# paplorinc/jtokkit

Hardware: AMD Instinct MI355X
Metric: input MB/s encoded (cl100k_base), HBM-resident input and output, bit-exact vs CPU oracle (higher is better)
Workload: dtype int32; 1 GPU; cl100k_base, 1M mixed UTF-8 docs (emoji + CJK, ~4 KB each); docs=1000000, bytes=4099377688, docs_per_gpu=1000000, bytes_per_gpu=4099377688, encode=encode() incl. the special-token check

## Files before the change

### jtokkit_amd/csrc/jtk_kernels.hip

```cpp
#include "jtk_kernels.h"

#include <type_traits>

#include "jtk_device_prims.h"
#include "jtk_merge_core.h"
#include "jtk_merge_order_rules.h"
#include "jtk_block_classify.h"
#include "jtk_split_masks.h"
#include "jtk_split_rules.h"

namespace {

constexpr int WAVE = 64;

__device__ __forceinline__ uint64_t lanemask_lt() {
    const unsigned lane = threadIdx.x & 63u;
    return (1ull << lane) - 1ull;
}

__device__ __forceinline__ void wave_lds_fence() {
    __builtin_amdgcn_fence(__ATOMIC_RELEASE, "wavefront");
    __builtin_amdgcn_wave_barrier();
    __builtin_amdgcn_fence(__ATOMIC_ACQUIRE, "wavefront");
}
// ... 1213 lines not shown
        uint32_t r = JTK_RANK_NONE;
        if (lane == 0 && nn >= 0) r = jtk_pair_lookup(pt, minr, ids[nn]);
        if (lane == 1 && pv >= 0) r = jtk_pair_lookup(pt, ids[pv], minr);
        wave_lds_fence();
        if (lane == 0) { ids[mini] = minr; rk[mini] = r; ids[nxt] = JTK_ID_DEAD; }
        if (lane == 1 && pv >= 0) rk[pv] = r;
        wave_lds_fence();
    }
}

template <int CAP>
__device__ __forceinline__ void merge_long(const JtkWork& w, const JtkDeviceTables& t, uint32_t* s_id, uint32_t* s_rk,
                                           uint32_t wave_id, uint32_t n_waves) {
    const int lane = threadIdx.x & 63;
    const JtkLongPiece* list = (CAP == JTK_MID_CAP) ? w.mid_list : w.long_list;
    const uint32_t cnt = (CAP == JTK_MID_CAP) ? *w.mid_count : *w.long_count;
    for (uint32_t i = wave_id; i < cnt; i += n_waves) {
        const JtkLongPiece lp = list[i];
        if (lp.len <= 0) continue;
        const int len = (int)lp.len;
        for (int j = lane; j < len; j += WAVE) {
            const uint32_t b0 = w.text[lp.start + j];
            s_id[j] = t.byte_rank[b0];
            s_rk[j] = (j + 1 < len) ? t.bp_rank[(b0 << 8) | w.text[lp.start + j + 1]] : JTK_RANK_NONE;
        }
        wave_lds_fence();
        merge_piece_wave(s_id, s_rk, len, t.pairs);
        uint32_t total = 0;
        for (int base = 0; base < len; base += WAVE) {
            const int j = base + lane;
            const bool alive = j < len && s_id[j] != JTK_ID_DEAD;
            const uint64_t bal = __ballot(alive);
            const uint32_t idx = total + (uint32_t)__popcll(bal & lanemask_lt());
            if (alive && idx) w.htok[lp.start + idx] = s_id[j];
            total += (uint32_t)__popcll(bal);
        }
        if (lane == 0) {
            w.htok[lp.start] = s_id[0] | (total << JTK_HT_CNT_SHIFT);
            atomicAdd(&w.tile_tot[lp.start / T], total);
        }
        wave_lds_fence();
    }
}

__device__ __forceinline__ uint64_t wave_min_u64(uint64_t v) {
#pragma unroll
    for (int d = 1; d < 64; d <<= 1) {
        const uint32_t lo = (uint32_t)__shfl_xor((int)(uint32_t)v, d), hi = (uint32_t)__shfl_xor((int)(uint32_t)(v >> 32), d);
        const uint64_t o = ((uint64_t)hi << 32) | lo;
        v = o < v ? o : v;
    }
    return v;
}

struct GiantLds {
    uint64_t* cmin;
    uint64_t* wmin;
    int* nb;
    uint32_t* r;
};

__device__ void merge_giant(const JtkWork& w, const JtkDeviceTables& t, const GiantLds& L, uint32_t gi) {
    constexpr int CH = JTK_GIANT_CHUNK;
    const int tid = threadIdx.x, lane = tid & 63, wv = tid >> 6, NT = blockDim.x, NWV = NT >> 6;
    const JtkLongPiece lp = w.giant_list[gi];
    if (lp.len <= 0) return;
    const int len = (int)lp.len;
    uint32_t* gid = w.htok + lp.start;
    uint32_t* grk = w.docpre + lp.start;
    const int nch = (len + CH - 1) / CH;
    constexpr uint64_t KNONE = ~0ull;

    for (int j = tid; j < len; j += NT) {
        const uint32_t b0 = w.text[lp.start + j];
        gid[j] = t.byte_rank[b0];
        grk[j] = (j + 1 < len) ? t.bp_rank[(b0 << 8) | w.text[lp.start + j + 1]] : JTK_RANK_NONE;
    }
    __syncthreads();
    auto chunk_min = [&](int c) {
        uint64_t k = KNONE;
        for (int q = 0; q < CH / 64; q++) {
            const int j = c * CH + q * 64 + lane;
            if (j < len) { const uint32_t r = grk[j]; if (r != JTK_RANK_NONE) { const uint64_t kk = ((uint64_t)r << 20) | (uint32_t)j; k = kk < k ? kk : k; } }
        }
        k = wave_min_u64(k);
        if (lane == 0) L.cmin[c] = k;
    };
    for (int c = wv; c < nch; c += NWV) chunk_min(c);
    __syncthreads();

    for (;;) {
        uint64_t k = KNONE;
        for (int c = tid; c < nch; c += NT) { const uint64_t kk = L.cmin[c]; k = kk < k ? kk : k; }
        k = wave_min_u64(k);
        if (lane == 0) L.wmin[wv] = k;
        __syncthreads();
        k = L.wmin[0];
        for (int q = 1; q < NWV; q++) k = L.wmin[q] < k ? L.wmin[q] : k;
        if (k == KNONE) break;
        const uint32_t minr = (uint32_t)(k >> 20);
        const int mini = (int)(k & 0xFFFFFu);
        if (wv == 0) {
            int nxt = -1, nn = -1;
            for (int base = mini + 1; base < len && nn < 0; base += WAVE) {
                const int j = base + lane;
                uint64_t bal = __ballot(j < len && gid[j] != JTK_ID_DEAD);
                if (nxt < 0 && bal) { nxt = base + jtk_ctz64(bal); bal &= bal - 1; }
                if (nxt >= 0 && bal) nn = base + jtk_ctz64(bal);
            }
            if (lane == 0) { L.nb[0] = nxt; L.nb[1] = nn; L.r[0] = nn >= 0 ? jtk_pair_lookup(t.pairs, minr, gid[nn]) : JTK_RANK_NONE; }
        } else if (wv == 1) {
            int pv = -1;
            for (int base = mini - 1; base >= 0 && pv < 0; base -= WAVE) {
                const int j = base - lane;
                const uint64_t bal = __ballot(j >= 0 && gid[j] != JTK_ID_DEAD);
                if (bal) pv = base - jtk_ctz64(bal);
            }
            if (lane == 0) { L.nb[2] = pv; L.r[1] = pv >= 0 ? jtk_pair_lookup(t.pairs, gid[pv], minr) : JTK_RANK_NONE; }
        }
        __syncthreads();
        const int nxt = L.nb[0], pv = L.nb[2];
        if (tid == 0) {
            gid[mini] = minr; grk[mini] = L.r[0];
            gid[nxt] = JTK_ID_DEAD; grk[nxt] = JTK_RANK_NONE;
            if (pv >= 0) grk[pv] = L.r[1];
        }
        __syncthreads();
        const int c0 = mini / CH, c1 = nxt / CH, c2 = pv >= 0 ? pv / CH : c0;
        if (wv == 0) chunk_min(c0);
        if (wv == 1 && c1 != c0) chunk_min(c1);
        if (wv == 2 && c2 != c0 && c2 != c1) chunk_min(c2);
        __syncthreads();
    }
    if (wv == 0) {
        uint32_t total = 0;
        uint32_t first = 0;
        for (int base = 0; base < len; base += WAVE) {
            const int j = base + lane;
            const uint32_t v = j < len ? gid[j] : JTK_ID_DEAD;
            const bool alive = v != JTK_ID_DEAD;
            const uint64_t bal = __ballot(alive);
            const uint32_t idx = total + (uint32_t)__popcll(bal & lanemask_lt());
            if (base == 0) first = (uint32_t)__shfl((int)v, 0);
            if (alive && idx) gid[idx] = v;
            total += (uint32_t)__popcll(bal);
        }
        if (lane == 0) {
            gid[0] = first | ((uint32_t)JTK_HT_ESCAPE << JTK_HT_CNT_SHIFT);
            grk[1] = total;
            atomicAdd(&w.tile_tot[lp.start / T], total);
        }
    }
    __syncthreads();
}

__global__ void __launch_bounds__(ML_THREADS) k_bpe_merge(JtkWork w, JtkDeviceTables t) {
    __shared__ alignas(16) uint32_t s_id[ML_WORDS];
    __shared__ alignas(16) uint32_t s_rk[ML_WORDS];
    __shared__ uint64_t s_bpbits[1024];
    __shared__ uint32_t s_bpranks[JTK_BP_MAX];
    __shared__ uint16_t s_bpcum[1024];
    __shared__ uint32_t s_brank[256];
    __shared__ uint32_t s_next[JTK_NBINS];
    __shared__ uint32_t s_count[JTK_NBINS + 3];
    __shared__ uint32_t s_ntiny;
    const int tid = threadIdx.x;
    const int shard = blockIdx.x % JTK_Q_SHARDS;
    const uint32_t kq = blockIdx.x / JTK_Q_SHARDS;
    if (tid < JTK_NBINS) {
        s_next[tid] = 0;
        s_count[tid] = w.q_count[JTK_QC(tid, shard)];
    }
    if (tid == 16) s_ntiny = w.q_count[JTK_QC(JTK_BIN_TINY, shard)];
    if (tid == JTK_NBINS) s_count[JTK_NBINS] = *w.mid_count;
    if (tid == JTK_NBINS + 1) s_count[JTK_NBINS + 1] = *w.long_count;
    if (tid == JTK_NBINS + 2) s_count[JTK_NBINS + 2] = *w.n_giant;
    __syncthreads();
    const uint32_t n0 = s_count[0], n1 = s_count[1], n2 = s_count[2], n3 = s_count[3], n4 = s_count[4];
    const uint32_t nt5 = s_ntiny;
    const bool rest = (s_count[5] | s_count[6] | s_count[JTK_NBINS] | s_count[JTK_NBINS + 1] | s_count[JTK_NBINS + 2]) != 0u;
    const bool side_by_side = n0 <= (uint32_t)ML_THREADS && n1 <= (uint32_t)ML_THREADS && n2 <= (uint32_t)ML_THREADS &&
                              nt5 <= (uint32_t)ML_THREADS && n3 <= (uint32_t)(ML_THREADS / 2) && n4 <= (uint32_t)(ML_THREADS / 4) &&
                              gridDim.x / JTK_Q_SHARDS >= 4u;
    const uint32_t K = side_by_side ? 1u : gridDim.x / JTK_Q_SHARDS, k = side_by_side ? 0u : kq;
    bool w0, w1, w2, w3, w4, w5;
    if (side_by_side) {
        w0 = kq == 0u && n0; w1 = kq == 1u && n1; w2 = kq == 2u && n2;
        w5 = kq == 3u && nt5; w3 = kq == 3u && n3; w4 = kq == 3u && n4;
    } else {
        w0 = kq * (uint32_t)ML_THREADS < n0; w1 = kq * (uint32_t)ML_THREADS < n1; w2 = kq * (uint32_t)ML_THREADS < n2;
        w3 = kq * (uint32_t)(ML_THREADS / 2) < n3; w4 = kq * (uint32_t)(ML_THREADS / 4) < n4;
        w5 = kq * (uint32_t)ML_THREADS < nt5;
    }
    if (!(w0 || w1 || w2 || w3 || w4 || w5 || rest)) return;
    for (int i = tid; i < 1024; i += ML_THREADS) { s_bpbits[i] = t.bp.bits[i]; s_bpcum[i] = t.bp.cum[i]; }
    for (int i = tid; i < JTK_BP_MAX; i += ML_THREADS) s_bpranks[i] = t.bp.ranks[i];
    if (tid < 256) s_brank[tid] = t.byte_rank[tid];
    __syncthreads();
    const LeanLds LL{s_id, s_rk, JtkBpLds{s_bpbits, s_bpcum, s_bpranks}, s_brank};
    if (w5) tiny_bin<ML_THREADS>(w, LL, nt5, k, K);
    if (w0) lean_bin<16, ML_THREADS, 0>(w, t, LL, n0, k, K);
    if (w1) lean_bin<16, ML_THREADS, 1>(w, t, LL, n1, k, K);
    if (w2) lean_bin<16, ML_THREADS, 2>(w, t, LL, n2, k, K);
    if (w3) { __syncthreads(); lean_bin<32, ML_THREADS / 2, 3>(w, t, LL, n3, k, K); }
    if (w4) { __syncthreads(); lean_bin<64, ML_THREADS / 4, 4>(w, t, LL, n4, k, K); }
    if (!rest) return;
    const MergeLds L{s_id, s_rk, s_bpbits, s_bpranks, s_bpcum, s_brank, s_next, s_count};
    if (s_count[5]) { __syncthreads(); merge_bin<128, ML_WORDS / 128, 5>(w, t, L); }
    if (s_count[6]) { __syncthreads(); merge_bin<256, ML_WORDS / 256, 6>(w, t, L); }
    const uint32_t wv = (uint32_t)tid >> 6;
    if (s_count[JTK_NBINS]) {
        __syncthreads();
        merge_long<JTK_MID_CAP>(w, t, s_id + wv * JTK_MID_CAP, s_rk + wv * JTK_MID_CAP, blockIdx.x * (uint32_t)(ML_THREADS / 64) + wv,
                                gridDim.x * (uint32_t)(ML_THREADS / 64));
    }
    if (s_count[JTK_NBINS + 1]) {
        __syncthreads();
        if (wv == 0) merge_long<JTK_LONG_CAP>(w, t, s_id, s_rk, blockIdx.x, gridDim.x);
    }
    if (s_count[JTK_NBINS + 2]) {
        __syncthreads();
        const GiantLds G{reinterpret_cast<uint64_t*>(s_id), reinterpret_cast<uint64_t*>(s_rk), reinterpret_cast<int*>(s_rk + 64),
                         s_rk + 72};
        for (uint32_t gi = blockIdx.x; gi < s_count[JTK_NBINS + 2]; gi += gridDim.x) merge_giant(w, t, G, gi);
    }
}

constexpr int SCAN_CHUNK = 4096;

__global__ void __launch_bounds__(1024) k_tile_scan(JtkWork w) {
    __shared__ uint64_t s_part[16];
    __shared__ uint32_t s_wsum[16];
    const int tid = threadIdx.x, lane = tid & 63, wv = tid >> 6;
    const int64_t chunk = blockIdx.x;
    uint64_t b = 0;
    {
        const int64_t nb = chunk * SCAN_CHUNK;
        const uint4* t4 = reinterpret_cast<const uint4*>(w.tile_tot);
        for (int64_t i = tid; i < nb / 4; i += 1024) { const uint4 v = t4[i]; b += (uint64_t)v.x + v.y + v.z + v.w; }
    }
    for (int d = 32; d >= 1; d >>= 1) {
        const uint32_t lo = (uint32_t)__shfl_xor((int)(uint32_t)b, d), hi = (uint32_t)__shfl_xor((int)(uint32_t)(b >> 32), d);
        b += ((uint64_t)hi << 32) | lo;
    }
    if (lane == 0) s_part[wv] = b;
    const int64_t i0 = chunk * SCAN_CHUNK + (int64_t)tid * 4;
    uint32_t v[4];
    uint32_t sum = 0;
    for (int j = 0; j < 4; j++) { v[j] = (i0 + j < w.n_tiles) ? w.tile_tot[i0 + j] : 0u; sum += v[j]; }
    const uint32_t inc = jtk_wave_incl_scan(sum);
    if (lane == 63) s_wsum[wv] = inc;
    __syncthreads();
    const uint64_t job_before = (uint64_t)*w.job_tokens;
    uint64_t before = job_before;
    for (int k = 0; k < 16; k++) before += s_part[k];
    for (int k = 0; k < wv; k++) before += s_wsum[k];
    uint64_t run = before + inc - sum;
    for (int j = 0; j < 4; j++) { if (i0 + j < w.n_tiles) w.tile_off[i0 + j] = (int64_t)run; run += v[j]; }
    if (chunk == gridDim.x - 1 && tid == 1023) {
        w.tile_off[w.n_tiles] = (int64_t)run;
        w.set_info[0] = (int64_t)job_before;
        w.set_info[1] = (int64_t)run;
        w.result->n_tokens = (int64_t)run;
        *w.job_tokens_next = (int64_t)run;
    }
}

__device__ __forceinline__ uint32_t hard_count(const JtkWork& w, int64_t pos) {
    const uint32_t c = (w.htok[pos] >> JTK_HT_CNT_SHIFT) & JTK_HT_CNT_MASK;
    if (c != JTK_HT_ESCAPE) return c;
    return w.docpre[pos + 1];
}

template <typename P> __device__ __forceinline__ P* uniform_ptr(P* p) {
    const uint64_t v = reinterpret_cast<uint64_t>(p);
    return reinterpret_cast<P*>((uint64_t)(uint32_t)__builtin_amdgcn_readfirstlane((int)(uint32_t)v) |
                                (uint64_t)(uint32_t)__builtin_amdgcn_readfirstlane((int)(uint32_t)(v >> 32)) << 32);
}

struct __attribute__((packed, aligned(4))) U4Unaligned { uint32_t x, y, z, w; };
__device__ __forceinline__ void pack_copy(uint32_t* dst, const uint32_t* src, uint32_t c) {
    for (uint32_t i = 0; i < c; i += 8) {
        const U4Unaligned a = *reinterpret_cast<const U4Unaligned*>(src + i), b = *reinterpret_cast<const U4Unaligned*>(src + i + 4);
        dst[i] = a.x & JTK_HT_ID_MASK;
        if (i + 1 < c) dst[i + 1] = a.y & JTK_HT_ID_MASK;
        if (i + 2 < c) dst[i + 2] = a.z & JTK_HT_ID_MASK;
        if (i + 3 < c) dst[i + 3] = a.w & JTK_HT_ID_MASK;
        if (i + 4 < c) dst[i + 4] = b.x & JTK_HT_ID_MASK;
        if (i + 5 < c) dst[i + 5] = b.y & JTK_HT_ID_MASK;
        if (i + 6 < c) dst[i + 6] = b.z & JTK_HT_ID_MASK;
        if (i + 7 < c) dst[i + 7] = b.w & JTK_HT_ID_MASK;
    }
}

template <int I> __device__ __forceinline__ uint32_t res_tok(const uint4& r) {
    constexpr int bit = 17 * I, wd = bit / 32, sh = bit % 32;
    const uint32_t w0 = wd == 0 ? r.x : wd == 1 ? r.y : wd == 2 ? r.z : r.w;
    const uint32_t w1 = wd == 0 ? r.y : wd == 1 ? r.z : r.w;
    return (sh + 17 <= 32 ? (w0 >> sh) : __builtin_amdgcn_alignbit(w1, w0, sh)) & JTK_HT_ID_MASK;
}

constexpr int PACK_STAGE = JTK_PACK_STAGE;
constexpr int PQT = JTK_PACK_TINY;

__global__ void __launch_bounds__(64) k_pack_tokens(JtkWork w) {
    __shared__ uint4 s_qe[JTK_PACK_SLOTS + JTK_PACK_OUT_SLOTS];
    __shared__ uint2 s_qt[PQT];
    __shared__ uint64_t s_dm[TW];
    __shared__ uint32_t s_ext[8];
    uint32_t* const s_out = reinterpret_cast<uint32_t*>(s_qe + JTK_PACK_SLOTS);
    const int lane = threadIdx.x;
    const int64_t tile = blockIdx.x;
    const int64_t B = tile * T;
    const int np = (int)w.tile_np[tile];
    const uint32_t total = w.tile_tot[tile];
    const uint32_t meta = lane < 16 ? w.q_meta[tile * 16 + lane] : 0u;
    const bool stage = total <= (uint32_t)PACK_STAGE;
    const bool store = w.count_only == 0;
    const uint32_t* plist = w.plist + B;
    int64_t tile_base;
    if (w.inline_scan) {
        uint32_t part = 0;
        for (int64_t i = lane; i < tile; i += 64) part += w.tile_tot[i];
#pragma unroll
        for (int d = 32; d >= 1; d >>= 1) part += (uint32_t)__shfl_xor((int)part, d);
        const int64_t job_before = *w.job_tokens;
        tile_base = job_before + (int64_t)part;
        if (lane == 0) {
            w.tile_off[tile] = tile_base;
            if (tile == w.n_tiles - 1) {
                const int64_t end = tile_base + (int64_t)total;
                w.tile_off[w.n_tiles] = end;
                w.set_info[0] = job_before;
                w.set_info[1] = end;
                w.result->n_tokens = end;
                *w.job_tokens_next = end;
            }
        }
    } else tile_base = w.tile_off[tile];
    uint32_t* const dst = reinterpret_cast<uint32_t*>(w.tokens + tile_base);
    uint32_t e[8];
#pragma unroll
    for (int j = 0; j < 8; j++) e[j] = plist[j * 64 + lane];
    uint64_t dmw = 0ull;
    if (lane < TW) {
        const int64_t dwd = (B >> 6) + lane;
        if (dwd < w.n_words) dmw = w.docmask[dwd];
    }
    const int64_t shard = tile % JTK_Q_SHARDS;
    uint4 rh = make_uint4(0, 0, 0, 0), rl = make_uint4(0, 0, 0, 0);
    bool hv, lv = false;
    {
        const int bl = lane < 32 ? 0 : lane < 48 ? 1 : 2, il = lane < 32 ? lane : lane < 48 ? lane - 32 : lane - 48;
        const uint32_t qbv = (uint32_t)__shfl((int)meta, bl), nqv = (uint32_t)__shfl((int)meta, 8 + bl);
        const uint4* const p0 = uniform_ptr(w.qd[0] + shard * w.q_cap[0]), * const p1 = uniform_ptr(w.qd[1] + shard * w.q_cap[1]),
                   * const p2 = uniform_ptr(w.qd[2] + shard * w.q_cap[2]);
        const uint4* src = (bl == 0 ? p0 : bl == 1 ? p1 : p2) + qbv;
        hv = (uint32_t)il < nqv;
        if (hv) rh = src[il];
    }
    const uint32_t nq_hi = (uint32_t)__shfl((int)meta, 11) | (uint32_t)__shfl((int)meta, 12) | (uint32_t)__shfl((int)meta, 13) | (uint32_t)__shfl((int)meta, 14);
    if (nq_hi) {
        const int bq = 3 + ((lane >> 3) & 3), il = lane & 7;
        const uint32_t qb = (uint32_t)__shfl((int)meta, bq), nq = (uint32_t)__shfl((int)meta, 8 + bq);
        lv = lane < 32 && (uint32_t)il < nq;
        const uint4* const p3 = uniform_ptr(w.qd[3] + shard * w.q_cap[3]), * const p4 = uniform_ptr(w.qd[4] + shard * w.q_cap[4]),
                   * const p5 = uniform_ptr(w.qd[5] + shard * w.q_cap[5]), * const p6 = uniform_ptr(w.qd[6] + shard * w.q_cap[6]);
        if (lv) rl = ((bq == 3 ? p3 : bq == 4 ? p4 : bq == 5 ? p5 : p6) + qb)[il];
    }
    const uint32_t qb5 = (uint32_t)__shfl((int)meta, JTK_BIN_TINY), nq5 = (uint32_t)__shfl((int)meta, 8 + JTK_BIN_TINY);
    const uint2* const res5 = reinterpret_cast<const uint2*>(w.qt + shard * w.qt_cap + qb5);
    uint2 rt[PQT / 64];
    if (nq5) {
#pragma unroll
        for (int r = 0; r < PQT / 64; r++) {
            const uint32_t i = (uint32_t)(r * 64 + lane);
            rt[r] = make_uint2(0, 0);
            if (i < nq5) rt[r] = res5[i];
        }
    }
    constexpr int XR = JTK_PACK_OUT_SLOTS / 64;
    const uint32_t over = (lane >= 8 && lane < 8 + JTK_NBINS_STAGE) ? jtk_stage_over(lane - 8, meta) : 0u;
    const bool has_ext = __ballot(over != 0u) != 0ull;
    uint4 rx[XR];
    uint32_t xend = 0;
    const uint32_t x0 = (uint32_t)JTK_PACK_SLOTS + jtk_stage_first_free(total);
    if (has_ext) {
        const uint32_t inc = jtk_wave_incl_scan(over);
        uint32_t xoff, xn;
        jtk_stage_place(total, inc - over, over, &xoff, &xn);
        if (lane >= 8 && lane < 16) s_ext[lane - 8] = lane < 8 + JTK_NBINS_STAGE ? jtk_stage_word(lane - 8, xoff, xn) : 0u;
        xend = (uint32_t)__builtin_amdgcn_readlane((int)(xoff + xn), 8 + JTK_NBINS_STAGE - 1);
#pragma unroll
        for (int r = 0; r < XR; r++) {
            rx[r] = make_uint4(0, 0, 0, 0);
            if (x0 + r * 64 >= xend) break;
            const uint32_t slot = x0 + r * 64 + lane;
            const uint4* src = nullptr;
#pragma unroll
            for (int b = 0; b < JTK_NBINS_STAGE; b++) {
                const uint32_t n = (uint32_t)__builtin_amdgcn_readlane((int)xn, 8 + b);
                if (n == 0u) continue;
                const uint32_t o = (uint32_t)__builtin_amdgcn_readlane((int)xoff, 8 + b), qb = (uint32_t)__builtin_amdgcn_readlane((int)meta, b);
                const uint4* base = w.qd[b] + shard * w.q_cap[b] + qb + JTK_PACK_CAP(b);
                src = slot - o < n ? base + (slot - o) : src;
            }
            if (slot < xend) rx[r] = *src;
        }
    }
    if (lane < TW) s_dm[lane] = dmw;
    if (hv) s_qe[lane] = rh;
    if (nq_hi) { if (lv) s_qe[JTK_PACK_OFF(3) + lane] = rl; }
    if (nq5) {
#pragma unroll
        for (int r = 0; r < PQT / 64; r++) {
            const uint32_t i = (uint32_t)(r * 64 + lane);
            if (i < nq5) s_qt[i] = rt[r];
        }
    }
    if (has_ext) {
#pragma unroll
        for (int r = 0; r < XR; r++) {
            const uint32_t slot = x0 + r * 64 + lane;
            if (slot < xend) s_qe[slot] = rx[r];
        }
    }
#pragma unroll
    for (int j = 0; j < 8; j++) e[j] = (j * 64 + lane < np) ? e[j] : 0u;
    wave_lds_fence();
    uint32_t run = 0;
    auto tiny_word = [](uint2 r) { return make_uint4(r.x, r.y & 0x3FFFFFFFu, 0u, (r.y >> 30) << 24); };
#define STORE(x) do { if (store) { x; } } while (0)
    auto step = [&](uint32_t* out, uint32_t ej, int k) {
        const bool valid = k < np;
        const bool hard = (ej & JTK_PL_HARD) != 0;
        const uint32_t bin = (ej >> JTK_PL_BIN_SHIFT) & 7u, qi = (ej >> JTK_PL_QI_SHIFT) & 1023u;
        const bool queued = hard && !(ej & JTK_PL_NOQUEUE);
        const bool tinyp = bin == JTK_BIN_TINY;
        const bool staged = queued && (ej & JTK_PL_STAGED) != 0u;
        uint32_t sidx = staged && !tinyp ? qi : 0u;
        bool inlds = staged;
        if (has_ext) {
            const uint32_t xw = s_ext[bin];
            const bool x = queued && !staged && qi < (xw >> 16);
            sidx = x ? (xw & 0xFFFFu) + qi : sidx;
            inlds = staged || x;
        }
        uint4 qe = s_qe[sidx];
        if (__ballot(queued && tinyp)) { if (staged && tinyp) qe = tiny_word(s_qt[qi]); }
        uint32_t c = valid ? (hard ? (qe.w >> 24) + 1u : 1u) : 0u;
        const uint32_t off = hard ? (ej & 2047u) : ((ej >> JTK_PL_OFF_SHIFT) & 2047u);
        const bool isdoc = valid && ((s_dm[off >> 6] >> (off & 63)) & 1ull);
        uint32_t pre;
        if (!__ballot(valid && hard && (!inlds || c > 7u))) {
            const uint32_t x = c ? c - 1u : 0u;
            const uint64_t bv = __ballot(valid);
            const uint64_t b0 = __ballot((x & 1u) != 0u), b1 = __ballot((x & 2u) != 0u), b2 = __ballot((x & 4u) != 0u);
            auto below = [](uint64_t m, uint32_t acc) { return __builtin_amdgcn_mbcnt_hi((uint32_t)(m >> 32), __builtin_amdgcn_mbcnt_lo((uint32_t)m, acc)); };
            pre = below(b0, below(bv, run));
            run += (uint32_t)__popcll(bv) + (uint32_t)__popcll(b0);
            if (b1 | b2) {
                pre += 2u * below(b1, 0u) + 4u * below(b2, 0u);
                run += 2u * (uint32_t)__popcll(b1) + 4u * (uint32_t)__popcll(b2);
            }
            if (valid) STORE(out[pre] = (hard ? qe.x : ej) & JTK_HT_ID_MASK);
            if (b0 | b1 | b2) {
                if (c > 1u) STORE(out[pre + 1] = res_tok<1>(qe));
                if (c > 2u) STORE(out[pre + 2] = res_tok<2>(qe));
                if (b1 | b2) {
                    if (c > 3u) STORE(out[pre + 3] = res_tok<3>(qe));
                    if (b2) {
                        if (c > 4u) STORE(out[pre + 4] = res_tok<4>(qe));
                        if (c > 5u) STORE(out[pre + 5] = res_tok<5>(qe));
                        if (c > 6u) STORE(out[pre + 6] = res_tok<6>(qe));
                    }
                }
            }
        } else {
            const uint32_t qb = (uint32_t)__shfl((int)meta, (int)(bin < JTK_NBINS ? bin : 0u));
            if (valid && queued && !inlds) {
                qe = tinyp ? tiny_word(res5[qi]) : (w.qd[bin] + shard * w.q_cap[bin] + qb)[qi];
                c = (qe.w >> 24) + 1u;
            } else if (valid && hard && !queued) c = hard_count(w, B + off);
            const uint32_t inc = jtk_wave_incl_scan(c);
            pre = run + inc - c;
            run += (uint32_t)__shfl((int)inc, 63);
            if (valid) {
                if (!hard) STORE(out[pre] = ej & JTK_HT_ID_MASK);
                else if (queued && c <= 7u) {
                    STORE(out[pre] = qe.x & JTK_HT_ID_MASK);
                    if (c > 1u) STORE(out[pre + 1] = res_tok<1>(qe));
                    if (c > 2u) STORE(out[pre + 2] = res_tok<2>(qe));
                    if (c > 3u) STORE(out[pre + 3] = res_tok<3>(qe));
                    if (c > 4u) STORE(out[pre + 4] = res_tok<4>(qe));
                    if (c > 5u) STORE(out[pre + 5] = res_tok<5>(qe));
                    if (c > 6u) STORE(out[pre + 6] = res_tok<6>(qe));
                } else if (store) pack_copy(out + pre, w.htok + B + off, c);
            }
        }
        if (__ballot(isdoc)) { if (isdoc) w.docpre[B + off] = pre; }
    };
#undef STORE
    for (int k0 = 0; k0 < np; k0 += 512) {
        if (k0) {
#pragma unroll
            for (int j = 0; j < 8; j++) { const int k = k0 + j * 64 + lane; e[j] = (k < np) ? plist[k] : 0u; }
        }
#pragma unroll
        for (int j = 0; j < 8; j++) {
            if (k0 + j * 64 >= np) break;
            if (stage) step(s_out, e[j], k0 + j * 64 + lane);
            else step(dst, e[j], k0 + j * 64 + lane);
        }
    }
    if (stage && store) {
        wave_lds_fence();
        for (uint32_t i = lane; i < total; i += WAVE) dst[i] = s_out[i];
    }
}

__global__ void __launch_bounds__(256) k_doc_offsets(JtkWork w) {
    const int64_t d = (int64_t)blockIdx.x * blockDim.x + threadIdx.x;
    if (d > w.n_docs) return;
    const int64_t q = w.doc_off[d] - w.text_base;
    w.tok_off[d] = (q >= w.n_bytes || q < w.lead) ? w.tile_off[w.n_tiles] : w.tile_off[q / T] + w.docpre[q];
    if (d < w.n_docs) {
        const int32_t st = w.status[d];
        if (st < 0) atomicMin(&w.result->worst_status, st);
    }
}

__device__ uint32_t long_lookup(const JtkWork& w, const JtkDeviceTables& t, int64_t pos, int64_t len) {
    if (len > (int64_t)t.longtok.max_len || len <= 16) return JTK_RANK_NONE;
    uint64_t h = JTK_FNV_BASIS;
    for (int64_t j = 0; j < len; j++) h = jtk_fnv1a_step(h, w.text[pos + j]);
    const uint32_t n = t.longtok.n;
    for (uint32_t i = (uint32_t)(h % n), probes = 0; probes < n; i = (i + 1) % n, probes++) {
        const JtkLongTokSlot sl = t.longtok.slots[i];
        if (sl.len == 0) return JTK_RANK_NONE;
        if (sl.h_lo == (uint32_t)h && sl.h_hi == (uint32_t)(h >> 32) && sl.len == (uint32_t)len) {
            bool eq = true;
            for (int64_t j = 0; j < len && eq; j++) eq = t.longtok.blob[sl.blob_off + j] == w.text[pos + j];
            if (eq) return sl.id;
        }
    }
    return JTK_RANK_NONE;
}

__global__ void __launch_bounds__(256) k_long_shortcut(JtkWork w, JtkDeviceTables t) {
    const uint32_t gtid = blockIdx.x * blockDim.x + threadIdx.x, gn = gridDim.x * blockDim.x;
    for (int bin = JTK_NBINS_BYTES; bin < JTK_NBINS; bin++) {
        for (int shard = 0; shard < JTK_Q_SHARDS; shard++) {
            const uint32_t count = w.q_count[JTK_QC(bin, shard)];
            uint64_t* qm = w.qm[bin] + (int64_t)shard * w.q_cap[bin];
            uint4* qd = w.qd[bin] + (int64_t)shard * w.q_cap[bin];
            for (uint32_t i = gtid; i < count; i += gn) {
                const uint64_t meta = qm[i];
                const int64_t pos = (int64_t)(meta & JTK_QE_POS_MASK);
                const uint32_t id = long_lookup(w, t, pos, (int64_t)((meta >> JTK_QE_LEN_SHIFT) & 255u) + 1);
                if (id != JTK_RANK_NONE) {
                    qd[i] = make_uint4(id, 0u, 0u, 0u);
                    qm[i] = meta | JTK_QE_DONE;
                    atomicAdd(&w.tile_tot[pos / T], 1u);
                }
            }
        }
    }
    for (int which = 0; which < 3; which++) {
        JtkLongPiece* list = which == 0 ? w.mid_list : which == 1 ? w.long_list : w.giant_list;
        const uint32_t count = which == 0 ? *w.mid_count : which == 1 ? *w.long_count : *w.n_giant;
        for (uint32_t i = gtid; i < count; i += gn) {
            const JtkLongPiece lp = list[i];
            const uint32_t id = long_lookup(w, t, lp.start, lp.len);
            if (id != JTK_RANK_NONE) {
                w.htok[lp.start] = id | (1u << JTK_HT_CNT_SHIFT);
                list[i].len = 0;
                atomicAdd(&w.tile_tot[lp.start / T], 1u);
            }
        }
    }
}

}

__global__ void __launch_bounds__(256) k_plan_chunks(const int64_t* doc_off, int64_t n_docs, int64_t chunk_bytes, int n_chunks,
                                                     int64_t* out_doc, int64_t* out_off) {
    const int c = (int)(blockIdx.x * blockDim.x + threadIdx.x);
    if (c > n_chunks) return;
    const int64_t lo = c == n_chunks ? n_docs : jtk_first_ge(doc_off, 0, n_docs, (int64_t)c * chunk_bytes);
    out_doc[c] = lo;
    out_off[c] = doc_off[lo];
}

void jtk_launch_plan_chunks(const int64_t* doc_off, int64_t n_docs, int64_t chunk_bytes, int n_chunks, int64_t* out_doc, int64_t* out_off,
                            hipStream_t s) {
    hipLaunchKernelGGL(k_plan_chunks, dim3((unsigned)((n_chunks + 1 + 255) / 256)), dim3(256), 0, s, doc_off, n_docs, chunk_bytes, n_chunks,
                       out_doc, out_off);
}

__global__ void __launch_bounds__(256) k_stitch(const int64_t* totals, int rank, int64_t* base_out, const int64_t* tok_off, int64_t n_docs,
                                                int64_t* global_off) {
    int64_t base = 0;
    for (int r = 0; r < rank; r++) base += totals[r];
    const int64_t d = (int64_t)blockIdx.x * blockDim.x + threadIdx.x;
    if (d == 0) *base_out = base;
    if (global_off && d <= n_docs) global_off[d] = tok_off[d] + base;
}
void jtk_launch_stitch(const int64_t* totals, int rank, int64_t* base_out, const int64_t* tok_off, int64_t n_docs, int64_t* global_off,
                       hipStream_t s) {
    const int64_t n = global_off ? n_docs + 1 : 1;
    hipLaunchKernelGGL(k_stitch, dim3((unsigned)((n + 255) / 256)), dim3(256), 0, s, totals, rank, base_out, tok_off, n_docs, global_off);
}

__global__ void __launch_bounds__(256) k_mark_pieces(JtkWork w, const int64_t* begin, const int64_t* end, int64_t n_pieces) {
    const int64_t i = (int64_t)blockIdx.x * blockDim.x + threadIdx.x;
    if (i >= n_pieces) return;
    const int64_t p = begin[i] - w.text_base, e = end[i] - w.text_base;
    if (p < w.lead || e <= p || e > w.n_bytes || (i + 1 < n_pieces && begin[i + 1] - w.text_base < e)) {
        atomicMin(&w.result->worst_status, -1 );
        return;
    }
    atomicOr((unsigned long long*)&w.piecemask[p >> 6], 1ull << (p & 63));
    const bool next_adjacent = (i + 1 < n_pieces) && (begin[i + 1] - w.text_base == e);
    if (!next_adjacent && e < w.n_bytes) {
        atomicOr((unsigned long long*)&w.piecemask[e >> 6], 1ull << (e & 63));
        atomicOr((unsigned long long*)&w.gapmask[e >> 6], 1ull << (e & 63));
    }
}
__global__ void __launch_bounds__(256) k_mark_doc_gaps(JtkWork w) {
    const int64_t d = (int64_t)blockIdx.x * blockDim.x + threadIdx.x;
    if (d > w.n_docs) return;
    const int64_t q = w.doc_off[d] - w.text_base;
    if (q < w.lead || q > w.n_bytes) return;
    const uint64_t bit = 1ull << (q & 63);
    const uint64_t old = atomicOr((unsigned long long*)&w.piecemask[q >> 6], bit);
    if (!(old & bit) && q < w.n_bytes) atomicOr((unsigned long long*)&w.gapmask[q >> 6], bit);
}
void jtk_launch_mark_pieces(const JtkWork& w, const int64_t* begin, const int64_t* end, int64_t n_pieces, hipStream_t s) {
    if (n_pieces > 0)
        hipLaunchKernelGGL(k_mark_pieces, dim3((unsigned)((n_pieces + 255) / 256)), dim3(256), 0, s, w, begin, end, n_pieces);
    const int64_t n = w.n_docs + 1;
    hipLaunchKernelGGL(k_mark_doc_gaps, dim3((unsigned)((n + 255) / 256)), dim3(256), 0, s, w);
}

void jtk_launch_mark_docs(const JtkWork& w, hipStream_t s) {
    const int64_t n = w.n_docs + 1;
    hipLaunchKernelGGL(k_mark_docs, dim3((unsigned)((n + 255) / 256)), dim3(256), 0, s, w);
}
void jtk_launch_validate_utf8(const JtkWork& w, hipStream_t s) {
    if (w.n_bytes == 0) return;
    hipLaunchKernelGGL(k_validate_utf8, dim3((unsigned)((w.n_bytes + 255) / 256)), dim3(256), 0, s, w);
}
void jtk_launch_pretok_split(const JtkWork& w, const JtkDeviceTables& t, hipStream_t s) {
    const int64_t tiles = (w.n_bytes + 1 + SPLIT_BYTES - 1) / SPLIT_BYTES;
    if (t.kind == JTK_PAT_CL100K) hipLaunchKernelGGL(k_pretok_split<JTK_PAT_CL100K>, dim3((unsigned)tiles), dim3(SPLIT_THREADS), 0, s, w, t);
    else hipLaunchKernelGGL(k_pretok_split<JTK_PAT_R50K>, dim3((unsigned)tiles), dim3(SPLIT_THREADS), 0, s, w, t);
}
void jtk_launch_piece_resolve(const JtkWork& w, const JtkDeviceTables& t, hipStream_t s) {
    hipLaunchKernelGGL(k_piece_resolve, dim3((unsigned)w.n_tiles), dim3(RES_THREADS), 0, s, w, t);
}
void jtk_launch_long_shortcut(const JtkWork& w, const JtkDeviceTables& t, hipStream_t s) {
    if (t.longtok.n) hipLaunchKernelGGL(k_long_shortcut, dim3(256), dim3(256), 0, s, w, t);
}
void jtk_launch_bpe_merge(const JtkWork& w, const JtkDeviceTables& t, hipStream_t s) {
    hipLaunchKernelGGL(k_bpe_merge, dim3(JTK_Q_SHARDS * ML_WGS_PER_SHARD), dim3(ML_THREADS), 0, s, w, t);
}
void jtk_launch_tile_scan(const JtkWork& w, hipStream_t s) {
    hipLaunchKernelGGL(k_tile_scan, dim3((unsigned)((w.n_tiles + SCAN_CHUNK - 1) / SCAN_CHUNK)), dim3(1024), 0, s, w);
}
void jtk_launch_pack(const JtkWork& w, hipStream_t s) {
    hipLaunchKernelGGL(k_pack_tokens, dim3((unsigned)w.n_tiles), dim3(64), 0, s, w);
}
__global__ void __launch_bounds__(256) k_flag_unencodable(JtkWork w, uint32_t pseudo_base) {
    const int64_t t0 = w.tile_off[0], t1 = w.tile_off[w.n_tiles];
    const int64_t i = t0 + (int64_t)blockIdx.x * blockDim.x + threadIdx.x;
    if (i >= t1 || (uint32_t)w.tokens[i] < pseudo_base) return;
    const int64_t d = jtk_first_gt(w.tok_off, 1, w.n_docs, i) - 1;
    atomicMin(&w.status[d], -12 );
    atomicMin(&w.result->worst_status, -12);
}

void jtk_launch_flag_unencodable(const JtkWork& w, uint32_t pseudo_base, hipStream_t s) {
    if (w.n_bytes == 0) return;
    hipLaunchKernelGGL(k_flag_unencodable, dim3((unsigned)((w.n_bytes + 255) / 256)), dim3(256), 0, s, w, pseudo_base);
}

void jtk_launch_doc_offsets(const JtkWork& w, hipStream_t s) {
    const int64_t n = w.n_docs + 1;
    hipLaunchKernelGGL(k_doc_offsets, dim3((unsigned)((n + 255) / 256)), dim3(256), 0, s, w);
}
```

Measured before the change: 149,300 MB/s.

## Restructure pack kernel step: uniform tile base, split LDS reads, prefetch next plist round

Makes the tile base scalar with readfirstlane and replaces the ballot-guarded uint4 LDS read with two uint2 reads from either the tiny or extended queue, padding s_qt by one entry. The docmask probe now reads 32-bit words and is skipped when the tile has no doc starts. The outer loop prefetches the next 512 plist entries before processing the last slot of the current round, and restructures the store branches. It also inserts explicit vmcnt(0) waits after the slow path and after each prefetch, which may serialize outstanding stores and reduce memory-level parallelism.

After: 155,300 MB/s, median of 6. +4.0%, better.

```diff
diff --git a/jtokkit_amd/csrc/jtk_kernels.hip b/jtokkit_amd/csrc/jtk_kernels.hip
--- a/jtokkit_amd/csrc/jtk_kernels.hip
+++ b/jtokkit_amd/csrc/jtk_kernels.hip
@@ -1539,10 +1539,11 @@
 
 constexpr int PACK_STAGE = JTK_PACK_STAGE;
 constexpr int PQT = JTK_PACK_TINY;
+constexpr int WAITCNT_VMCNT0_GFX9 = 0x0F70;
 
 __global__ void __launch_bounds__(64) k_pack_tokens(JtkWork w) {
     __shared__ uint4 s_qe[JTK_PACK_SLOTS + JTK_PACK_OUT_SLOTS];
-    __shared__ uint2 s_qt[PQT];
+    __shared__ uint2 s_qt[PQT + 1];
     __shared__ uint64_t s_dm[TW];
     __shared__ uint32_t s_ext[8];
     uint32_t* const s_out = reinterpret_cast<uint32_t*>(s_qe + JTK_PACK_SLOTS);
@@ -1575,6 +1576,8 @@
             }
         }
     } else tile_base = w.tile_off[tile];
+    tile_base = (int64_t)((uint64_t)(uint32_t)__builtin_amdgcn_readfirstlane((int)(uint32_t)tile_base) |
+                          (uint64_t)(uint32_t)__builtin_amdgcn_readfirstlane((int)(uint32_t)((uint64_t)tile_base >> 32)) << 32);
     uint32_t* const dst = reinterpret_cast<uint32_t*>(w.tokens + tile_base);
     uint32_t e[8];
 #pragma unroll
@@ -1667,7 +1670,7 @@
     wave_lds_fence();
     uint32_t run = 0;
     auto tiny_word = [](uint2 r) { return make_uint4(r.x, r.y & 0x3FFFFFFFu, 0u, (r.y >> 30) << 24); };
-#define STORE(x) do { if (store) { x; } } while (0)
+    const bool anydoc = __ballot(dmw != 0ull) != 0ull;
     auto step = [&](uint32_t* out, uint32_t ej, int k) {
         const bool valid = k < np;
         const bool hard = (ej & JTK_PL_HARD) != 0;
@@ -1683,11 +1686,14 @@
             sidx = x ? (xw & 0xFFFFu) + qi : sidx;
             inlds = staged || x;
         }
-        uint4 qe = s_qe[sidx];
-        if (__ballot(queued && tinyp)) { if (staged && tinyp) qe = tiny_word(s_qt[qi]); }
+        const uint32_t off = hard ? (ej & 2047u) : ((ej >> JTK_PL_OFF_SHIFT) & 2047u);
+        const uint2* const rp = staged && tinyp ? s_qt + qi : reinterpret_cast<const uint2*>(s_qe + sidx);
+        const uint2 lo = rp[0], hi = rp[1];
+        uint32_t dm = 0u;
+        if (anydoc) dm = reinterpret_cast<const uint32_t*>(s_dm)[off >> 5];
+        uint4 qe = make_uint4(lo.x, lo.y, hi.x, hi.y);
+        if (staged && tinyp) qe = tiny_word(lo);
         uint32_t c = valid ? (hard ? (qe.w >> 24) + 1u : 1u) : 0u;
-        const uint32_t off = hard ? (ej & 2047u) : ((ej >> JTK_PL_OFF_SHIFT) & 2047u);
-        const bool isdoc = valid && ((s_dm[off >> 6] >> (off & 63)) & 1ull);
         uint32_t pre;
         if (!__ballot(valid && hard && (!inlds || c > 7u))) {
             const uint32_t x = c ? c - 1u : 0u;
@@ -1700,16 +1706,20 @@
                 pre += 2u * below(b1, 0u) + 4u * below(b2, 0u);
                 run += 2u * (uint32_t)__popcll(b1) + 4u * (uint32_t)__popcll(b2);
             }
-            if (valid) STORE(out[pre] = (hard ? qe.x : ej) & JTK_HT_ID_MASK);
-            if (b0 | b1 | b2) {
-                if (c > 1u) STORE(out[pre + 1] = res_tok<1>(qe));
-                if (c > 2u) STORE(out[pre + 2] = res_tok<2>(qe));
-                if (b1 | b2) {
-                    if (c > 3u) STORE(out[pre + 3] = res_tok<3>(qe));
-                    if (b2) {
-                        if (c > 4u) STORE(out[pre + 4] = res_tok<4>(qe));
-                        if (c > 5u) STORE(out[pre + 5] = res_tok<5>(qe));
-                        if (c > 6u) STORE(out[pre + 6] = res_tok<6>(qe));
+            if (store) {
+                char* const p = reinterpret_cast<char*>(out) + (size_t)(pre * 4u);
+                auto put = [&](int i, uint32_t v) { *reinterpret_cast<uint32_t*>(p + 4 * i) = v; };
+                if (valid) put(0, (hard ? qe.x : ej) & JTK_HT_ID_MASK);
+                if (b0 | b1 | b2) {
+                    if (c > 1u) put(1, res_tok<1>(qe));
+                    if (b1 | b2) {
+                        if (c > 2u) put(2, res_tok<2>(qe));
+                        if (c > 3u) put(3, res_tok<3>(qe));
+                        if (b2) {
+                            if (c > 4u) put(4, res_tok<4>(qe));
+                            if (c > 5u) put(5, res_tok<5>(qe));
+                            if (c > 6u) put(6, res_tok<6>(qe));
+                        }
                     }
                 }
             }
@@ -1722,34 +1732,48 @@
             const uint32_t inc = jtk_wave_incl_scan(c);
             pre = run + inc - c;
             run += (uint32_t)__shfl((int)inc, 63);
-            if (valid) {
-                if (!hard) STORE(out[pre] = ej & JTK_HT_ID_MASK);
+            if (valid && store) {
+                if (!hard) out[pre] = ej & JTK_HT_ID_MASK;
                 else if (queued && c <= 7u) {
-                    STORE(out[pre] = qe.x & JTK_HT_ID_MASK);
-                    if (c > 1u) STORE(out[pre + 1] = res_tok<1>(qe));
-                    if (c > 2u) STORE(out[pre + 2] = res_tok<2>(qe));
-                    if (c > 3u) STORE(out[pre + 3] = res_tok<3>(qe));
-                    if (c > 4u) STORE(out[pre + 4] = res_tok<4>(qe));
-                    if (c > 5u) STORE(out[pre + 5] = res_tok<5>(qe));
-                    if (c > 6u) STORE(out[pre + 6] = res_tok<6>(qe));
-                } else if (store) pack_copy(out + pre, w.htok + B + off, c);
-            }
-        }
-        if (__ballot(isdoc)) { if (isdoc) w.docpre[B + off] = pre; }
+                    out[pre] = qe.x & JTK_HT_ID_MASK;
+                    if (c > 1u) out[pre + 1] = res_tok<1>(qe);
+                    if (c > 2u) out[pre + 2] = res_tok<2>(qe);
+                    if (c > 3u) out[pre + 3] = res_tok<3>(qe);
+                    if (c > 4u) out[pre + 4] = res_tok<4>(qe);
+                    if (c > 5u) out[pre + 5] = res_tok<5>(qe);
+                    if (c > 6u) out[pre + 6] = res_tok<6>(qe);
+                } else pack_copy(out + pre, w.htok + B + off, c);
+            }
+            __builtin_amdgcn_s_waitcnt(WAITCNT_VMCNT0_GFX9);
+        }
+        if (anydoc) {
+            const bool isdoc = valid && ((dm >> (off & 31u)) & 1u);
+            if (__ballot(isdoc)) { if (isdoc) w.docpre[B + off] = pre; }
+        }
     };
-#undef STORE
-    for (int k0 = 0; k0 < np; k0 += 512) {
-        if (k0) {
-#pragma unroll
-            for (int j = 0; j < 8; j++) { const int k = k0 + j * 64 + lane; e[j] = (k < np) ? plist[k] : 0u; }
-        }
-#pragma unroll
-        for (int j = 0; j < 8; j++) {
-            if (k0 + j * 64 >= np) break;
-            if (stage) step(s_out, e[j], k0 + j * 64 + lane);
-            else step(dst, e[j], k0 + j * 64 + lane);
-        }
-    }
+    auto rounds = [&](uint32_t* out) {
+        for (int k0 = 0;; k0 += 512) {
+#pragma unroll
+            for (int j = 0; j < 7; j++) {
+                if (k0 + j * 64 >= np) return;
+                step(out, e[j], k0 + j * 64 + lane);
+            }
+            if (k0 + 512 >= np) {
+                if (k0 + 448 < np) step(out, e[7], k0 + 448 + lane);
+                return;
+            }
+            const uint32_t* nl = plist + k0 + 512 + lane;
+            const uint32_t e7 = e[7];
+#pragma unroll
+            for (int i = 0; i < 8; i++) e[i] = nl[i * 64];
+            step(out, e7, k0 + 448 + lane);
+            __builtin_amdgcn_s_waitcnt(WAITCNT_VMCNT0_GFX9);
+#pragma unroll
+            for (int i = 0; i < 8; i++) e[i] = (k0 + 512 + i * 64 + lane < np) ? e[i] : 0u;
+        }
+    };
+    if (stage) rounds(s_out);
+    else rounds(dst);
     if (stage && store) {
         wave_lds_fence();
         for (uint32_t i = lane; i < total; i += WAVE) dst[i] = s_out[i];
```
